# Chen-Suyi/PointRegGPT

Measured on AMD Instinct MI355X. Metric: generated point-cloud pairs/sec (node), 128x128 depth, 1000-step DDNM, higher is better.
Workload: dtype bf16; 1 GPU; configs[2]: full pipeline (SE(3) z-buffer reproject + MaskUnet + DDNM sampler + MaskUnet + f64 unproject); batch_per_gpu=64, image_size=128, transitions=1000, sampler=ancestral-ddnm, unet_dim=64, streams=2, parallelism=scene-sharded x1, no collectives, hipgraph=one captured transition (U-Net + update), replayed per step

## Files before the change

include/prg.h:

```cpp
#ifndef PRG_H
#define PRG_H

#include <stddef.h>
#include <stdint.h>

#ifdef __cplusplus
extern "C" {
#endif

#define PRG_ABI_VERSION 1

enum {
  PRG_OK = 0,
  PRG_E_INVALID = -1,
  PRG_E_HIP = -2,
  PRG_E_NOMEM = -3,
  PRG_E_STATE = -4
};

enum { PRG_F32 = 0, PRG_BF16 = 1, PRG_MXFP8 = 2, PRG_F16X3 = 3 };

int prg_abi_version(void);
const char* prg_last_error(void);
int prg_device_info(char* name, size_t name_len, int* compute_units);
// ... 17 lines not shown
                      int B, int H, int W, float depth_unit, float clip_lo, float clip_hi, void* stream);

int prg_depth_augment(const float* depth, float* out, int B, int H, int W, void* stream);

int prg_apply_mask(const float* prob, const float* depth, const uint8_t* hit, float thr, float* depth_out,
                   uint8_t* hit_out, float* img_cond, int B, int H, int W, void* stream);

int prg_occlusion_filter(const float* depth, const uint8_t* mask, float* out, int B, int H, int W, float threshold,
                         void* stream);

int prg_overlap_counts(const double* pts, const int64_t* offsets, int n_pairs, int64_t max_cloud, double radius,
                       int32_t* counts, void* stream);


typedef struct prg_unet prg_unet;

typedef struct prg_unet_config {
  int32_t dim;
  int32_t n_levels;
  int32_t dim_mults[8];
  int32_t in_channels;
  int32_t conditional;
  int32_t param_cond_dim;
  int32_t groups;
  int32_t sigmoid_out;
} prg_unet_config;

int64_t prg_unet_param_count(const prg_unet_config* cfg);

int prg_unet_create(const prg_unet_config* cfg, const float* weights, int64_t n_floats, int dtype,
                    prg_unet** out);
int prg_unet_destroy(prg_unet* h);
int prg_unet_set_time_freqs(prg_unet* h, const float* freqs, int n);
int prg_unet_reserve(prg_unet* h, int B, int S);

int prg_unet_forward(prg_unet* h, const float* x, const int64_t* time, const float* param_cond, float* out,
                     int B, int S, void* stream);
int prg_maskunet_forward(prg_unet* h, const float* depth, float* prob, int B, int S, void* stream);

int prg_unet_set_taps(prg_unet* h, int enable);
int prg_unet_get_tap(prg_unet* h, const char* name, float* out, int64_t out_capacity_floats, int* C, int* H,
                     int* W, void* stream);

int prg_debug_conv3x3(const float* x, const float* w, const float* bias, float* out, int B, int Cin, int Cout, int H, int W,
                      int dtype, void* stream);
int prg_debug_block_pair(const float* x, const float* w1, const float* b1, const float* gamma, const float* beta, const float* w2,
                         const float* b2, float* out, int B, int Cin, int C, int H, int W, int groups, int h16, void* stream);
int prg_debug_upsample_conv3x3(const float* x, const float* w, const float* bias, float* out, int B, int Cin, int Cout, int H,
                               int W, void* stream);
int prg_debug_conv4x4s2(const float* x, const float* w, const float* bias, float* out, int B, int Cin, int Cout, int H, int W,
                        void* stream);
int prg_debug_conv(const float* x, const float* w, const float* bias, float* out, int B, int Cin, int Cout, int H, int W,
                   int dtype, int K, int stride, void* stream);
int prg_debug_upsample_conv(const float* x, const float* w, const float* bias, float* out, int B, int Cin, int Cout, int H, int W,
                            int dtype, void* stream);


typedef struct prg_sampler prg_sampler;

typedef struct prg_step {
  int32_t t;
  int32_t clip_pred;
  float c_x0, c_x, c_eps, sigma;
  float sqrt_recip, sqrt_recipm1;
} prg_step;

int prg_sampler_create(prg_unet* unet, const prg_step* steps, int n_steps, int B, int S, prg_sampler** out);
int prg_sampler_destroy(prg_sampler* h);
int prg_sampler_set_graph(prg_sampler* h, int enable);

int prg_sampler_run(prg_sampler* h, const float* param_cond, const float* img_cond, const float* noise,
                    int64_t noise_slabs, const uint64_t* seeds, float* out, void* stream);

int prg_debug_sampler_step(float* x, const float* u, const float* img_cond, const uint64_t* seeds, const prg_step* step, int B,
                           int HW, int reps, float* avg_us, void* stream);

int prg_sampler_set_profile(prg_sampler* h, int enable);
int prg_sampler_get_profile(prg_sampler* h, double* conv_ms, int64_t* conv_launches, double* conv_flops,
                            double* total_ms);
int prg_sampler_get_profile_bytes(prg_sampler* h, double* conv_bytes);
int prg_sampler_get_profile_executed(prg_sampler* h, double* conv_flops_executed);
typedef struct prg_profile_shape {
  int32_t cin, cout, k, stride, ups, hout, wout;
  int32_t two_source, prologue;
  int32_t mx;
  int64_t launches;
  double ms, flops, flops_executed;
} prg_profile_shape;
int prg_sampler_get_profile_shapes(prg_sampler* h, prg_profile_shape* rows, int32_t max_rows, int32_t* n_rows);
int prg_sampler_get_profile_step(prg_sampler* h, double* step_ms, int64_t* step_launches);


int prg_host_crop_aabb(const double* pts, int64_t n, const double* lo, const double* hi, double* out, int64_t* n_out);
int prg_host_voxel_down_sample(const double* pts, int64_t n, double voxel, double* out, int64_t* n_out);
int prg_host_write_ply(const char* path, const double* pts, int64_t n);

typedef struct prg_pool prg_pool;
int prg_pool_create(int n_threads, prg_pool** out);
int prg_pool_destroy(prg_pool* p);
int prg_pool_wait(prg_pool* p, int64_t* jobs_done);
int prg_pool_submit_cloud(prg_pool* p, const char* path, const double* xyz, int64_t n, const uint8_t* valid,
                          const double* T_pre, int crop, const double* lo, const double* hi, double voxel,
                          const double* T_post);
int prg_pool_submit_image(prg_pool* p, const char* path, const float* img, int H, int W, int kind);
int prg_pool_submit_text(prg_pool* p, const char* path, const double* values, int rows, int cols);

// ... 5 lines not shown
```

pointreggpt_amd/_lib.py:

```python
from __future__ import annotations

import ctypes as C
import os
from pathlib import Path

_HERE = Path(__file__).resolve().parent
LIB_PATH = Path(os.environ.get("PRG_HIP_LIB", _HERE / "libprg_hip.so"))

PRG_F32, PRG_BF16, PRG_MXFP8, PRG_F16X3 = 0, 1, 2, 3


class PrgError(RuntimeError):
    pass


class UnetConfigC(C.Structure):
    _fields_ = [("dim", C.c_int32), ("n_levels", C.c_int32), ("dim_mults", C.c_int32 * 8),
                ("in_channels", C.c_int32), ("conditional", C.c_int32), ("param_cond_dim", C.c_int32),
                ("groups", C.c_int32), ("sigmoid_out", C.c_int32)]


class StepC(C.Structure):
    _fields_ = [("t", C.c_int32), ("clip_pred", C.c_int32), ("c_x0", C.c_float), ("c_x", C.c_float),
                ("c_eps", C.c_float), ("sigma", C.c_float), ("sqrt_recip", C.c_float),
                ("sqrt_recipm1", C.c_float)]


_P, _I, _F, _L = C.c_void_p, C.c_int, C.c_float, C.c_int64

PROTOTYPES = {
    "prg_abi_version": (C.c_int, []),
    "prg_last_error": (C.c_char_p, []),
    "prg_device_info": (C.c_int, [C.c_char_p, C.c_size_t, C.POINTER(C.c_int)]),
    "prg_depth2pc": (C.c_int, [_P, _P, _P, _P, _I, _I, _I, _F, _F, _F, _P]),
    "prg_pc2depth": (C.c_int, [_P, _P, _P, _P, _P, _I, _I, _I, _I, _P]),
    "prg_project_points_zbuffer": (C.c_int, [_P, _P, _P, _P, _P, _P, _I, _I, _I, _F, _P]),
    "prg_reproject_zbuffer": (C.c_int, [_P, _P, _P, _P, _P, _I, _I, _I, _F, _F, _F, _F, _P]),
    "prg_unproject_f64": (C.c_int, [_P, _P, _P, _P, _P, _I, _I, _I, _F, _F, _F, _P]),
    "prg_depth_augment": (C.c_int, [_P, _P, _I, _I, _I, _P]),
    "prg_apply_mask": (C.c_int, [_P, _P, _P, _F, _P, _P, _P, _I, _I, _I, _P]),
    "prg_occlusion_filter": (C.c_int, [_P, _P, _P, _I, _I, _I, _F, _P]),
    "prg_overlap_counts": (C.c_int, [_P, _P, _I, _L, C.c_double, _P, _P]),
    "prg_unet_param_count": (_L, [C.POINTER(UnetConfigC)]),
    "prg_unet_create": (C.c_int, [C.POINTER(UnetConfigC), _P, _L, _I, C.POINTER(_P)]),
    "prg_unet_destroy": (C.c_int, [_P]),
    "prg_unet_reserve": (C.c_int, [_P, _I, _I]),
    "prg_unet_set_time_freqs": (C.c_int, [_P, _P, _I]),
    "prg_unet_forward": (C.c_int, [_P, _P, _P, _P, _P, _I, _I, _P]),
    "prg_maskunet_forward": (C.c_int, [_P, _P, _P, _I, _I, _P]),
    "prg_debug_conv3x3": (C.c_int, [_P, _P, _P, _P, _I, _I, _I, _I, _I, _I, _P]),
    "prg_debug_block_pair": (C.c_int, [_P, _P, _P, _P, _P, _P, _P, _P, _I, _I, _I, _I, _I, _I, _I, _P]),
    "prg_debug_upsample_conv3x3": (C.c_int, [_P, _P, _P, _P, _I, _I, _I, _I, _I, _P]),
    "prg_debug_conv4x4s2": (C.c_int, [_P, _P, _P, _P, _I, _I, _I, _I, _I, _P]),
    "prg_debug_conv": (C.c_int, [_P, _P, _P, _P, _I, _I, _I, _I, _I, _I, _I, _I, _P]),
    "prg_debug_upsample_conv": (C.c_int, [_P, _P, _P, _P, _I, _I, _I, _I, _I, _I, _P]),
    "prg_unet_set_taps": (C.c_int, [_P, _I]),
    "prg_unet_get_tap": (C.c_int, [_P, C.c_char_p, _P, _L, C.POINTER(_I), C.POINTER(_I), C.POINTER(_I), _P]),
    "prg_sampler_create": (C.c_int, [_P, C.POINTER(StepC), _I, _I, _I, C.POINTER(_P)]),
    "prg_sampler_destroy": (C.c_int, [_P]),
    "prg_sampler_set_graph": (C.c_int, [_P, _I]),
    "prg_sampler_run": (C.c_int, [_P, _P, _P, _P, _L, _P, _P, _P]),
    "prg_sampler_set_profile": (C.c_int, [_P, _I]),
    "prg_sampler_get_profile": (C.c_int, [_P, C.POINTER(C.c_double), C.POINTER(_L), C.POINTER(C.c_double),
                                          C.POINTER(C.c_double)]),
    "prg_sampler_get_profile_bytes": (C.c_int, [_P, C.POINTER(C.c_double)]),
    "prg_sampler_get_profile_executed": (C.c_int, [_P, C.POINTER(C.c_double)]),
    "prg_sampler_get_profile_step": (C.c_int, [_P, C.POINTER(C.c_double), C.POINTER(_L)]),
    "prg_debug_sampler_step": (C.c_int, [_P, _P, _P, _P, _P, C.c_int, C.c_int, C.c_int, C.POINTER(C.c_float), _P]),
    "prg_sampler_get_profile_shapes": (C.c_int, [_P, _P, _I, C.POINTER(C.c_int32)]),
    "prg_host_crop_aabb": (C.c_int, [_P, _L, _P, _P, _P, C.POINTER(_L)]),
    "prg_host_voxel_down_sample": (C.c_int, [_P, _L, C.c_double, _P, C.POINTER(_L)]),
    "prg_host_write_ply": (C.c_int, [C.c_char_p, _P, _L]),
    "prg_pool_create": (C.c_int, [_I, C.POINTER(_P)]),
    "prg_pool_destroy": (C.c_int, [_P]),
    "prg_pool_wait": (C.c_int, [_P, C.POINTER(_L)]),
    "prg_pool_submit_cloud": (C.c_int, [_P, C.c_char_p, _P, _L, _P, _P, _I, _P, _P, C.c_double, _P]),
    "prg_pool_submit_image": (C.c_int, [_P, C.c_char_p, _P, _I, _I, _I]),
    "prg_pool_submit_text": (C.c_int, [_P, C.c_char_p, _P, _I, _I]),
}

_lib = None


def load():
    global _lib
    if _lib is not None:
        return _lib
    import torch
    if not LIB_PATH.exists():
        raise PrgError(f"{LIB_PATH} not found: build it with `python -c 'import __graft_entry__ as g; g.build()'` "
                       f"or `make -C pointreggpt_amd/csrc` (there is no CPU fallback)")
    try:
        lib = C.CDLL(str(LIB_PATH))
    except OSError as e:
        raise PrgError(f"cannot load {LIB_PATH}: {e}") from e
    lenient = os.environ.get("PRG_HIP_LIB_ALLOW_MISSING", "0") not in ("", "0") and bool(os.environ.get("PRG_HIP_LIB"))
    for name, (res, args) in PROTOTYPES.items():
        if lenient and not hasattr(lib, name):
            continue
        fn = getattr(lib, name)
        fn.restype = res
        fn.argtypes = args
    if lib.prg_abi_version() != 1:
        raise PrgError(f"ABI version mismatch: library {lib.prg_abi_version()}, binding 1")
    _lib = lib
    return lib
# ... 25 lines not shown
```

pointreggpt_amd/csrc/conv.h:

```cpp
#pragma once
#include <vector>

#include "common.h"

namespace prg {

template <typename T>
struct ConvTile {
  static constexpr int BK = 64 / (int)sizeof(T);
};

struct ConvDesc {
  int B, Hin, Win;
  int C0, C1;
  int ups;
  int KH, KW, stride, pad;
  int Hout, Wout;
  int Cout, CoutPad;
  int kchunks;
};

template <typename T>
void pack_conv_weight(const float* w_oihw, int Cout, int Cin, int KH, int KW, std::vector<T>& out, int* CoutPad,
                      int* kchunks);
// ... 44 lines not shown
}
typedef __attribute__((ext_vector_type(4))) unsigned int h16_u32x4;
#define PRG_H16_TRANS4(OP)                                                                                             \
  asm(OP "_e32 %0, %4\n\t" OP "_e32 %1, %5\n\t" OP "_e32 %2, %6\n\t" OP "_e32 %3, %7\n\t"                            \
      OP "_sdwa %0, %4 dst_sel:WORD_1 dst_unused:UNUSED_PRESERVE src0_sel:WORD_1\n\t"                                  \
      OP "_sdwa %1, %5 dst_sel:WORD_1 dst_unused:UNUSED_PRESERVE src0_sel:WORD_1\n\t"                                  \
      OP "_sdwa %2, %6 dst_sel:WORD_1 dst_unused:UNUSED_PRESERVE src0_sel:WORD_1\n\t"                                  \
      OP "_sdwa %3, %7 dst_sel:WORD_1 dst_unused:UNUSED_PRESERVE src0_sel:WORD_1\n\ts_nop 0"                           \
      : "=&v"(o0), "=&v"(o1), "=&v"(o2), "=&v"(o3)                                                                      \
      : "v"(i0), "v"(i1), "v"(i2), "v"(i3))
__device__ inline h16_u32x4 h16_silu8(h16_u32x4 x, const h16x2 (&a)[4], const h16x2 (&b)[4]) {
  const h16x2 nl2e = {(_Float16)-1.4426950408889634f, (_Float16)-1.4426950408889634f}, one = {(_Float16)1.0f, (_Float16)1.0f};
  h16x2 y[4];
  uint32_t i0, i1, i2, i3, o0, o1, o2, o3;
#pragma unroll
  for (int j = 0; j < 4; ++j) {
    const uint32_t w = x[j];
    y[j] = __builtin_elementwise_fma(__builtin_bit_cast(h16x2, w), a[j], b[j]);
  }
  i0 = __builtin_bit_cast(uint32_t, y[0] * nl2e); i1 = __builtin_bit_cast(uint32_t, y[1] * nl2e);
  i2 = __builtin_bit_cast(uint32_t, y[2] * nl2e); i3 = __builtin_bit_cast(uint32_t, y[3] * nl2e);
  PRG_H16_TRANS4("v_exp_f16");
  i0 = __builtin_bit_cast(uint32_t, __builtin_bit_cast(h16x2, o0) + one); i1 = __builtin_bit_cast(uint32_t, __builtin_bit_cast(h16x2, o1) + one);
  i2 = __builtin_bit_cast(uint32_t, __builtin_bit_cast(h16x2, o2) + one); i3 = __builtin_bit_cast(uint32_t, __builtin_bit_cast(h16x2, o3) + one);
  PRG_H16_TRANS4("v_rcp_f16");
  h16_u32x4 r;
  r[0] = __builtin_bit_cast(uint32_t, y[0] * __builtin_bit_cast(h16x2, o0));
  r[1] = __builtin_bit_cast(uint32_t, y[1] * __builtin_bit_cast(h16x2, o1));
  r[2] = __builtin_bit_cast(uint32_t, y[2] * __builtin_bit_cast(h16x2, o2));
  r[3] = __builtin_bit_cast(uint32_t, y[3] * __builtin_bit_cast(h16x2, o3));
  return r;
}
#undef PRG_H16_TRANS4
#endif

void pack_conv_weight_f16(const float* w_oihw, int Cout, int Cin, int KH, int KW, std::vector<uint16_t>& out);
bool conv_h16_pair_ok(const ConvLaunch<bf16_t>& L1, const ConvLaunch<bf16_t>& L2);

void pack_conv_weight_split(const float* w_oihw, int Cout, int Cin, int KH, int KW, std::vector<uint16_t>& out, int* CoutPad,
                            int* kchunks32, std::vector<float>* oscale = nullptr);
int try_launch_conv_split(const ConvLaunch<float>& L, hipStream_t s, int* gn_nsplit_out);

void s2d_equivalent_weights(const float* w_oihw, int Cout, int Cin, std::vector<float>& out);
void up_equivalent_weights(const float* w_oihw, int Cout, int Cin, std::vector<float>& out);

void pack_conv_weight_mxfp8(const float* w_oihw, int Cout, int Cin, int KH, int KW, std::vector<uint8_t>& data,
                            std::vector<uint8_t>& scales, int* CoutPad, int* chunks64);
uint8_t f32_to_e4m3(float v);
float e4m3_to_f32(uint8_t b);

template <typename T>
int launch_conv(const ConvLaunch<T>& L, hipStream_t s, int* gn_nsplit_out, int* acc_done = nullptr);

template <typename T>
bool conv_supports_prologue(const ConvDesc& d);

double conv_last_exec_scale();
int conv_last_was_mx();

inline double conv_flops(const ConvDesc& d) {
  return 2.0 * (double)d.B * d.Hout * d.Wout * d.Cout * (double)(d.C0 + d.C1) * d.KH * d.KW;
}

bool stem_conv_mfma_supported(int Cin, int Cout, int H, int W);
int launch_stem_conv_mfma(const float* x, const bf16_t* wf, const float* bias, bf16_t* out, int B, int Cin, int H, int W, hipStream_t s);
void pack_stem_mfma_weights(const float* w, int Cin, std::vector<bf16_t>& out);
int launch_stem_conv_mfma_split(const float* x, const uint16_t* wf, const float* bias, const float* wscale, float* out, int B, int Cin,
                                int H, int W, hipStream_t s);
void pack_stem_mfma_weights_split(const float* w, int Cin, std::vector<uint16_t>& out, std::vector<float>& scale);
template <typename T>
int launch_stem_conv(const float* x, const float* wk, const float* bias, T* out, int B, int Cin, int H, int W,
                     int Cout, hipStream_t s);

template <typename T>
int launch_head_conv(const T* x, const float* w, const float* bias, float* out, int64_t M, int C, int sigmoid,
                     hipStream_t s);

}
```

pointreggpt_amd/csrc/conv.hip:

```cpp
#include <cmath>
#include <cstdio>
#include <cstring>
#include <type_traits>

#include "blocks.h"
#include "conv.h"
#include "conv_epi.h"

namespace prg {

template <typename T>
struct Mma;

template <>
struct Mma<bf16_t> {
  static constexpr int UNITS_PER_CALL = 2;
  using Frag = bf16x8;
  __device__ static inline int unit_of(int call, int hi) { return call * 2 + hi; }
  __device__ static inline Frag load(const void* p) { return *reinterpret_cast<const Frag*>(p); }
  __device__ static inline void mma(const Frag& a, const Frag& b, f32x16& c, int ) {
    c = __builtin_amdgcn_mfma_f32_32x32x16_bf16(a, b, c, 0, 0, 0);
  }
};

// ... 725 lines not shown
  int rc;
  if ((rc = materialize_prologue(L, s))) return rc;
  if (hp.TH == 8 && hp.TW == 32 && hp.BN == 64) rc = launch_mx<8, 32, 64>(L, s, fuse, gn_nsplit_out);
  else if (hp.TH == 4 && hp.TW == 32 && hp.BN == 128) rc = launch_mx<4, 32, 128>(L, s, fuse, gn_nsplit_out);
  else if (hp.TH == 8 && hp.TW == 16 && hp.BN == 128) rc = launch_mx<8, 16, 128>(L, s, fuse, gn_nsplit_out);
  else if (hp.TH == 8 && hp.TW == 16 && hp.BN == 64) rc = launch_mx<8, 16, 64>(L, s, fuse, gn_nsplit_out);
  else return 0;
  if (rc == PRG_OK) g_last_mx = 1;
  return rc == PRG_OK ? 1 : rc;
}
static int try_mx(ConvLaunch<float>&, hipStream_t, int*, int*) { return 0; }

int try_launch_conv3x3_ws(const ConvLaunch<bf16_t>& L, hipStream_t s, int* gn_nsplit_out, int* acc_done);
int try_launch_conv3x3_c64(const ConvLaunch<bf16_t>& L, hipStream_t s, int* gn_nsplit_out, int* acc_done);
int try_launch_conv3x3_w256(const ConvLaunch<bf16_t>& L, hipStream_t s, int* gn_nsplit_out, int* acc_done);
int try_launch_conv4x4s2_w256(const ConvLaunch<bf16_t>& L, hipStream_t s);
int try_launch_conv3x3_up_w256(const ConvLaunch<bf16_t>& L, hipStream_t s);
static inline int try_down(const ConvLaunch<bf16_t>& L, hipStream_t s) { return try_launch_conv4x4s2_w256(L, s); }
static inline int try_down(const ConvLaunch<float>&, hipStream_t) { return 0; }
static inline int try_ws(ConvLaunch<bf16_t>& L, hipStream_t s, int* n, int* acc_done) {
  int r = try_launch_conv3x3_c64(L, s, n, acc_done);
  if (r == 0 && L.d.ups && !L.gn_partials) {
    r = try_launch_conv3x3_up_w256(L, s);
    if (r == 1) g_last_exec_scale = 4.0 / 9.0;
  }
  if (r == 0) r = try_launch_conv3x3_w256(L, s, n, acc_done);
  if (r != 0) return r;
  const ConvDesc& d = L.d;
  if (L.pro_fold.acc && d.KH == 3 && d.KW == 3 && d.stride == 1 && d.pad == 1 && d.C0 % 64 == 0 && d.C1 % 64 == 0 && d.Cout % 64 == 0)
    if (int rc = materialize_prologue(L, s)) return rc;
  return try_launch_conv3x3_ws(L, s, n, acc_done);
}
static inline int try_ws(ConvLaunch<float>&, hipStream_t, int*, int*) { return 0; }
static inline int try_split(const ConvLaunch<float>& L, hipStream_t s, int* n) { return try_launch_conv_split(L, s, n); }
static inline int try_split(const ConvLaunch<bf16_t>&, hipStream_t, int*) { return 0; }

bool conv_h16_pair_ok(const ConvLaunch<bf16_t>& L1in, const ConvLaunch<bf16_t>& L2in) {
  static const int on = env_int("PRG_H16", 1);
  if (!on) return false;
  ConvLaunch<bf16_t> L1 = L1in, L2 = L2in;
  auto mx_takes = [](const ConvLaunch<bf16_t>& L) { return L.w_mx && (L.d.Cout % 128 == 0 || mx_pure_env() || L.mx_pure); };
  if (mx_takes(L1) || mx_takes(L2) || !L2.w_f16 || !L1.gn_acc || !L2.pro_fold.acc) return false;
  L1.probe = L2.probe = 1;
  L1.out_f16 = 1;
  L2.in_f16 = 1;
  int ns = 0, ad = 0;
  int r1 = try_launch_conv3x3_c64(L1, nullptr, &ns, &ad);
  if (r1 == 0) r1 = try_launch_conv3x3_w256(L1, nullptr, &ns, &ad);
  if (r1 == 0) r1 = try_launch_conv3x3_ws(L1, nullptr, &ns, &ad);
  if (r1 != 1 || !ad) return false;
  int r2 = try_launch_conv3x3_c64(L2, nullptr, &ns, &ad);
  if (r2 == 0) r2 = try_launch_conv3x3_w256(L2, nullptr, &ns, &ad);
  return r2 == 1;
}

template <typename T>
int launch_conv(const ConvLaunch<T>& Lin, hipStream_t s, int* gn_nsplit_out, int* acc_done) {
  g_last_exec_scale = 1.0;
  g_last_mx = 0;
  if (acc_done) *acc_done = 0;
  ConvLaunch<T> L = Lin;
  const ConvDesc& d = L.d;
  constexpr int VEC = Elem<T>::kVec;
  PRG_CHECK(L.src0 && L.w && L.out, "conv: null pointer");
  PRG_CHECK(d.C0 % VEC == 0 && d.C1 % VEC == 0, "conv: channel counts must be multiples of the 16-byte vector");
  PRG_CHECK(d.C1 == 0 || L.src1, "conv: second source missing");
  PRG_CHECK(!L.res_a || (L.residual && L.res_b && d.KH == 1 && d.KW == 1 && d.Cout % 8 == 0),
            "conv: the activated residual is a 1x1 (implicit-GEMM, wide epilogue) feature");
  PRG_CHECK(!L.res_fold.acc || (L.residual && d.KH == 1 && d.KW == 1 && d.Cout % 8 == 0 && L.res_fold.cpg % 8 == 0 &&
                                L.res_fold.G * L.res_fold.cpg == d.Cout && L.res_fold.P && L.res_fold.Q),
            "conv: the folded activated residual needs a 1x1 conv whose 8-channel vectors lie inside one GroupNorm group");
  PRG_CHECK(d.CoutPad % 64 == 0 && d.CoutPad >= d.Cout, "conv: bad CoutPad");
  const int64_t M64 = (int64_t)d.B * d.Hout * d.Wout;
  PRG_CHECK(M64 > 0 && M64 < (int64_t)1 << 31, "conv: M out of range");
  const int M = (int)M64;
  const int want_stats = L.gn_partials != nullptr;
  if (gn_nsplit_out) *gn_nsplit_out = 0;
  {
    const int r = try_mx(L, s, gn_nsplit_out, acc_done);
    if (r < 0) return r;
    if (r == 1) return PRG_OK;
  }
  {
    int r = try_ws(L, s, gn_nsplit_out, acc_done);
    if (r == 0 && !L.gn_partials) r = try_down(L, s);
    if (r < 0) return r;
    if (r == 1) return PRG_OK;
  }
  PRG_CHECK(!L.out_f16 && !L.in_f16, "conv: an h16 launch reached a kernel without the f16 format (conv_h16_pair_ok disagrees with the dispatch)");
  if (int rc = materialize_prologue(L, s)) return rc;
  {
    const int r = try_split(L, s, gn_nsplit_out);
    if (r < 0) return r;
    if (r == 1) return PRG_OK;
  }
  HaloPick<T> hp;
  if (pick_halo<T>(d, &hp)) {
    const int cpg = L.gn_groups > 0 ? d.Cout / L.gn_groups : 0;
    const int tiles = (d.Wout / hp.TW) * (d.Hout / hp.TH);
    const int fuse = want_stats && cpg % 8 == 0 && cpg <= hp.BN && tiles <= kGnMaxSplit;
    if (hp.TH == 8 && hp.TW == 32 && hp.BN == 64) return launch_halo<T, 8, 32, 64>(L, s, fuse, gn_nsplit_out);
    if (hp.TH == 4 && hp.TW == 32 && hp.BN == 128) return launch_halo<T, 4, 32, 128>(L, s, fuse, gn_nsplit_out);
    if (hp.TH == 8 && hp.TW == 16 && hp.BN == 128) return launch_halo<T, 8, 16, 128>(L, s, fuse, gn_nsplit_out);
    if (hp.TH == 8 && hp.TW == 16 && hp.BN == 64) return launch_halo<T, 8, 16, 64>(L, s, fuse, gn_nsplit_out);
  }
  PRG_CHECK(!L.pro_a, "conv: fused prologue requested on a shape the halo kernel does not cover");
  if constexpr (std::is_same<T, bf16_t>::value) {
    if (d.CoutPad % 128 == 0 && M % 256 == 0 && (int64_t)(M / 256) * (d.CoutPad / 128) >= (int64_t)2 * 256)
      return launch_igemm<T, 256, 128>(L, M, s, want_stats, gn_nsplit_out);
  }
  if (d.CoutPad % 128 == 0) return launch_igemm<T, 128, 128>(L, M, s, want_stats, gn_nsplit_out);
  if (M >= 256 * 64) return launch_igemm<T, 256, 64>(L, M, s, want_stats, gn_nsplit_out);
  return launch_igemm<T, 128, 64>(L, M, s, want_stats, gn_nsplit_out);
}

void up_equivalent_weights(const float* w, int Cout, int Cin, std::vector<float>& out) {
  out.assign((size_t)4 * Cout * Cin * 4, 0.0f);
  auto slot = [](int dphase, int k) { const int r = dphase + k - 1; return (r >= 0 ? r / 2 : -1) - (dphase - 1); };
  for (int dy = 0; dy < 2; ++dy)
    for (int dx = 0; dx < 2; ++dx)
      for (int o = 0; o < Cout; ++o)
        for (int c = 0; c < Cin; ++c) {
          double acc[2][2] = {{0, 0}, {0, 0}};
          for (int ky = 0; ky < 3; ++ky)
            for (int kx = 0; kx < 3; ++kx) acc[slot(dy, ky)][slot(dx, kx)] += (double)w[(((size_t)o * Cin + c) * 3 + ky) * 3 + kx];
          float* dst = out.data() + ((((size_t)(2 * dy + dx) * Cout + o) * Cin + c) * 4);
          dst[0] = (float)acc[0][0]; dst[1] = (float)acc[0][1]; dst[2] = (float)acc[1][0]; dst[3] = (float)acc[1][1];
        }
}

void s2d_equivalent_weights(const float* w, int Cout, int Cin, std::vector<float>& out) {
  out.assign((size_t)Cout * 4 * Cin * 9, 0.0f);
  for (int o = 0; o < Cout; ++o)
    for (int c = 0; c < Cin; ++c)
      for (int ky = 0; ky < 4; ++ky)
        for (int kx = 0; kx < 4; ++kx) {
          const int by = ky >> 1, dy = ky & 1, bx = kx >> 1, dx = kx & 1;
          const int cv = (2 * dy + dx) * Cin + c;
          out[(((size_t)o * 4 * Cin + cv) * 3 + 1 + by) * 3 + 1 + bx] = w[(((size_t)o * Cin + c) * 4 + ky) * 4 + kx];
        }
}

template int launch_conv<float>(const ConvLaunch<float>&, hipStream_t, int*, int*);
template int launch_conv<bf16_t>(const ConvLaunch<bf16_t>&, hipStream_t, int*, int*);

template <typename T>
void pack_conv_weight(const float* w, int Cout, int Cin, int KH, int KW, std::vector<T>& out, int* CoutPad,
                      int* kchunks) {
  constexpr int BK = ConvTile<T>::BK;
  const int cp = (Cout + 63) / 64 * 64;
  const int kcn = (Cin + BK - 1) / BK;
  out.assign((size_t)KH * KW * kcn * cp * BK, Elem<T>::store(0.0f));
  for (int kh = 0; kh < KH; ++kh)
    for (int kw = 0; kw < KW; ++kw)
      for (int kc = 0; kc < kcn; ++kc)
        for (int n = 0; n < Cout; ++n)
          for (int k = 0; k < BK; ++k) {
            int c = kc * BK + k;
            if (c >= Cin) break;
            float v = w[(((size_t)n * Cin + c) * KH + kh) * KW + kw];
            out[((((size_t)(kh * KW + kw)) * kcn + kc) * cp + n) * BK + k] = Elem<T>::store(v);
          }
  *CoutPad = cp;
  *kchunks = kcn;
}
template void pack_conv_weight<float>(const float*, int, int, int, int, std::vector<float>&, int*, int*);
// ... 362 lines not shown
```

pointreggpt_amd/csrc/unet.hip:

```cpp
#include <algorithm>
#include <cmath>
#include <cstdlib>
#include <cstring>
#include <map>
#include <memory>
#include <string>
#include <type_traits>
#include <vector>

#include "blocks.h"
#include "conv.h"
#include "sampler.h"

namespace prg {

static thread_local std::string g_err;
void set_error(const std::string& m) { g_err = m; }
int device_cu_count() {
  static std::atomic<int> cus[64];
  int dev = 0;
  if (hipGetDevice(&dev) != hipSuccess) return 0;
  std::atomic<int>& c = cus[dev & 63];
  int n = c.load(std::memory_order_acquire);
  if (n <= 0) {
// ... 1551 lines not shown
  L1.src0 = reinterpret_cast<const bf16_t*>(d_x); L1.w = reinterpret_cast<const bf16_t*>(d_w1); L1.bias = reinterpret_cast<const float*>(d_b1);
  L1.out = reinterpret_cast<bf16_t*>(d_h);
  L1.gn_partials = reinterpret_cast<float*>(d_part); L1.gn_acc = reinterpret_cast<long long*>(d_acc);
  desc(L2, C, cp2, kc2);
  L2.src0 = reinterpret_cast<const bf16_t*>(d_h); L2.w = reinterpret_cast<const bf16_t*>(d_w2); L2.w_f16 = reinterpret_cast<const uint16_t*>(d_w2h);
  L2.bias = reinterpret_cast<const float*>(d_b2); L2.out = reinterpret_cast<bf16_t*>(d_y);
  GnFold f{};
  f.acc = reinterpret_cast<const long long*>(d_acc); f.P = reinterpret_cast<const float*>(d_pq); f.Q = f.P + C; f.pq_stride = 0;
  f.G = groups; f.cpg = C / groups; f.inv_n = 1.0f / ((float)(H * W) * (float)f.cpg);
  L2.pro_fold = f;
  L2.pro_a = reinterpret_cast<const float*>(d_coef); L2.pro_b = L2.pro_a + (size_t)B * C;
  if (rc == PRG_OK && h16) {
    if (!conv_h16_pair_ok(L1, L2)) rc = fail(PRG_E_INVALID, "prg_debug_block_pair: the kernels this shape dispatches to do not implement the f16 format");
    L1.out_f16 = 1;
    L2.in_f16 = 1;
  }
  int ns = 0, ad = 0;
  if (rc == PRG_OK) rc = launch_conv<bf16_t>(L1, s, &ns, &ad);
  if (rc == PRG_OK && !ad) rc = fail(PRG_E_INVALID, "prg_debug_block_pair: conv1's kernel does not accumulate fixed-point statistics for this shape");
  if (rc == PRG_OK) rc = launch_conv<bf16_t>(L2, s, nullptr);
  if (rc == PRG_OK) rc = launch_nhwc_to_nchw_f32<bf16_t>(reinterpret_cast<const bf16_t*>(d_y), out, B, H * W, C, s);
  if (hipStreamSynchronize(s) != hipSuccess && rc == PRG_OK) rc = fail(PRG_E_HIP, "prg_debug_block_pair: stream synchronise failed");
  cleanup();
  return rc;
}

int prg_debug_conv3x3(const float* x, const float* w, const float* bias, float* out, int B, int Cin, int Cout, int H, int W,
                      int dtype, void* stream) {
  return debug_conv(x, w, bias, out, B, Cin, Cout, H, W, dtype, 3, 1, stream);
}

int prg_debug_conv(const float* x, const float* w, const float* bias, float* out, int B, int Cin, int Cout, int H, int W,
                   int dtype, int K, int stride, void* stream) {
  PRG_CHECK((K == 1 || K == 3 || K == 4) && (stride == 1 || stride == 2), "prg_debug_conv: K must be 1, 3 or 4, stride 1 or 2");
  PRG_CHECK(dtype == PRG_F32 || dtype == PRG_F16X3 || K != 1, "prg_debug_conv: 1x1 convs only in the float32-storage modes");
  PRG_CHECK(stride == 1 || (H % 2 == 0 && W % 2 == 0), "prg_debug_conv: odd image size");
  return debug_conv(x, w, bias, out, B, Cin, Cout, H, W, dtype, K, stride, stream);
}

int prg_debug_upsample_conv3x3(const float* x, const float* w, const float* bias, float* out, int B, int Cin, int Cout, int H, int W,
                               void* stream) {
  return debug_conv(x, w, bias, out, B, Cin, Cout, H, W, PRG_BF16, 3, 1, stream, 1);
}

int prg_debug_upsample_conv(const float* x, const float* w, const float* bias, float* out, int B, int Cin, int Cout, int H, int W,
                            int dtype, void* stream) {
  return debug_conv(x, w, bias, out, B, Cin, Cout, H, W, dtype, 3, 1, stream, 1);
}

int prg_debug_conv4x4s2(const float* x, const float* w, const float* bias, float* out, int B, int Cin, int Cout, int H, int W,
                        void* stream) {
  PRG_CHECK(H % 2 == 0 && W % 2 == 0, "prg_debug_conv4x4s2: odd image size");
  return debug_conv(x, w, bias, out, B, Cin, Cout, H, W, PRG_BF16, 4, 2, stream);
}

int prg_sampler_create(prg_unet* unet, const prg_step* steps, int n_steps, int B, int S, prg_sampler** out) {
  PRG_CHECK(unet && steps && out, "prg_sampler_create: null pointer");
  PRG_CHECK(unet->lay.cfg.conditional && unet->lay.cfg.in_channels == 1, "prg_sampler_create: needs the conditional U-Net");
  PRG_CHECK(n_steps > 0 && B > 0 && S > 0, "prg_sampler_create: bad sizes");
  int rc = reserve(unet, B, S);
  if (rc) return rc;
  std::unique_ptr<prg_sampler> h(new prg_sampler());
  h->unet = unet; h->B = B; h->S = S; h->n_steps = n_steps;
  h->steps.assign(steps, steps + n_steps);
  const Layout& L = unet->lay;
  const int e = L.emb, d0 = L.cfg.dim, W = L.ss_total;
  const size_t HW = (size_t)S * S;
  const int R = n_steps > B ? n_steps : B;
  if (hipMalloc(&h->d_steps, sizeof(prg_step) * n_steps) != hipSuccess ||
      hipMalloc(&h->d_tpart, sizeof(float) * (size_t)n_steps * W) != hipSuccess ||
      hipMalloc(&h->d_ppart, sizeof(float) * (size_t)B * W) != hipSuccess ||
      hipMalloc(&h->d_scratch, sizeof(float) * (size_t)R * (d0 + 2 * e) + sizeof(int32_t) * n_steps) != hipSuccess ||
      hipMalloc(&h->d_x, sizeof(float) * B * HW) != hipSuccess || hipMalloc(&h->d_u, sizeof(float) * B * HW) != hipSuccess ||
      hipMalloc(&h->d_step, 2 * sizeof(int)) != hipSuccess || hipMalloc(&h->d_seeds, sizeof(uint64_t) * B) != hipSuccess)
    return fail(PRG_E_NOMEM, "prg_sampler_create: hipMalloc failed");
  PRG_HIP(hipMemcpy(h->d_steps, steps, sizeof(prg_step) * n_steps, hipMemcpyHostToDevice));
  PRG_HIP(hipStreamCreateWithFlags(&h->own_stream, hipStreamDefault));
  {
    hipStream_t s = h->own_stream;
    float* sinu = h->d_scratch;
    float* h1 = sinu + (size_t)R * d0;
    float* temb = h1 + (size_t)R * e;
    int32_t* tdev = reinterpret_cast<int32_t*>(temb + (size_t)R * e);
    std::vector<int32_t> tt(n_steps);
    for (int k = 0; k < n_steps; ++k) tt[k] = steps[k].t;
    PRG_HIP(hipMemcpyAsync(tdev, tt.data(), sizeof(int32_t) * n_steps, hipMemcpyHostToDevice, s));
    const float* F = unet->d_flat;
    if ((rc = launch_sinusoidal_i32(tdev, unet->d_freqs, sinu, n_steps, d0, s))) return rc;
    if ((rc = launch_linear(sinu, d0, 0, F + L.tm1_w, d0, 0, F + L.tm1_b, h1, e, n_steps, d0, e, ACT_NONE, ACT_GELU, s))) return rc;
    if ((rc = launch_linear(h1, e, 0, F + L.tm3_w, e, 0, F + L.tm3_b, temb, e, n_steps, e, e, ACT_NONE, ACT_NONE, s))) return rc;
    auto one = [&](const ResP& r) -> int {
      return launch_linear(temb, e, 0, F + r.mlp_w, 2 * e, 0, F + r.mlp_b, h->d_tpart + r.ss_off, W, n_steps, e,
                           2 * r.cout, ACT_SILU, ACT_NONE, s);
    };
    for (auto& lv : L.downs) { if ((rc = one(lv.r0))) return rc; if ((rc = one(lv.r1))) return rc; }
    for (auto& lv : L.ups) { if ((rc = one(lv.r0))) return rc; if ((rc = one(lv.r1))) return rc; }
    if ((rc = one(L.mid1))) return rc;
    if ((rc = one(L.mid2))) return rc;
    if ((rc = one(L.fin))) return rc;
    PRG_HIP(hipStreamSynchronize(s));
  }
  *out = h.release();
  return PRG_OK;
}

int prg_sampler_destroy(prg_sampler* h) {
// ... 161 lines not shown
```

Measured before the change: 14.49 pairs/s.

## Add dedicated async-LDS MFMA GEMM kernel for 1x1 convolutions

Adds a specialised bf16 GEMM kernel for 1x1 stride-1 convolutions, including two-source concatenated inputs. It uses global_load_lds double buffering into swizzled LDS, 32x32x16 MFMA tiles, and a fused bias/residual/GN-SiLU epilogue. The conv dispatcher tries it before the generic implicit-GEMM path when enough tiles exist and no stats or prologue are needed, aiming to cut the im2col-style overhead of the generic kernel on 1x1 shapes. A debug entry point is added to compare both paths. The risk is lower occupancy from 64KB of LDS, and coverage is limited to shapes whose channel counts are multiples of 64 and 128.

```diff
diff --git a/include/prg.h b/include/prg.h
--- a/include/prg.h
+++ b/include/prg.h
@@ -93,6 +93,8 @@
                         void* stream);
 int prg_debug_conv(const float* x, const float* w, const float* bias, float* out, int B, int Cin, int Cout, int H, int W,
                    int dtype, int K, int stride, void* stream);
+int prg_debug_conv1x1(const float* x0, const float* x1, const float* w, const float* bias, const float* residual, const float* res_ab,
+                      float* out, int B, int C0, int C1, int Cout, int H, int W, int path, void* stream);
 int prg_debug_upsample_conv(const float* x, const float* w, const float* bias, float* out, int B, int Cin, int Cout, int H, int W,
                             int dtype, void* stream);
 
diff --git a/pointreggpt_amd/_lib.py b/pointreggpt_amd/_lib.py
--- a/pointreggpt_amd/_lib.py
+++ b/pointreggpt_amd/_lib.py
@@ -52,6 +52,7 @@
     "prg_debug_block_pair": (C.c_int, [_P, _P, _P, _P, _P, _P, _P, _P, _I, _I, _I, _I, _I, _I, _I, _P]),
     "prg_debug_upsample_conv3x3": (C.c_int, [_P, _P, _P, _P, _I, _I, _I, _I, _I, _P]),
     "prg_debug_conv4x4s2": (C.c_int, [_P, _P, _P, _P, _I, _I, _I, _I, _I, _P]),
+    "prg_debug_conv1x1": (C.c_int, [_P, _P, _P, _P, _P, _P, _P, _I, _I, _I, _I, _I, _I, _I, _P]),
     "prg_debug_conv": (C.c_int, [_P, _P, _P, _P, _I, _I, _I, _I, _I, _I, _I, _I, _P]),
     "prg_debug_upsample_conv": (C.c_int, [_P, _P, _P, _P, _I, _I, _I, _I, _I, _I, _P]),
     "prg_unet_set_taps": (C.c_int, [_P, _I]),
diff --git a/pointreggpt_amd/csrc/conv.h b/pointreggpt_amd/csrc/conv.h
--- a/pointreggpt_amd/csrc/conv.h
+++ b/pointreggpt_amd/csrc/conv.h
@@ -120,6 +120,8 @@
 template <typename T>
 int launch_conv(const ConvLaunch<T>& L, hipStream_t s, int* gn_nsplit_out, int* acc_done = nullptr);
 
+int launch_conv1x1_path(const ConvLaunch<bf16_t>& L, hipStream_t s, int path);
+
 template <typename T>
 bool conv_supports_prologue(const ConvDesc& d);
 
diff --git a/pointreggpt_amd/csrc/conv.hip b/pointreggpt_amd/csrc/conv.hip
--- a/pointreggpt_amd/csrc/conv.hip
+++ b/pointreggpt_amd/csrc/conv.hip
@@ -801,6 +801,20 @@
   int r2 = try_launch_conv3x3_c64(L2, nullptr, &ns, &ad);
   if (r2 == 0) r2 = try_launch_conv3x3_w256(L2, nullptr, &ns, &ad);
   return r2 == 1;
+}
+
+int try_launch_conv_gemm(const ConvLaunch<bf16_t>& L, hipStream_t s, int force);
+
+template <typename T>
+static int launch_generic_igemm(const ConvLaunch<T>& L, int M, hipStream_t s, int want_stats, int* gn_nsplit_out) {
+  const ConvDesc& d = L.d;
+  if constexpr (std::is_same<T, bf16_t>::value) {
+    if (d.CoutPad % 128 == 0 && M % 256 == 0 && (int64_t)(M / 256) * (d.CoutPad / 128) >= (int64_t)2 * 256)
+      return launch_igemm<T, 256, 128>(L, M, s, want_stats, gn_nsplit_out);
+  }
+  if (d.CoutPad % 128 == 0) return launch_igemm<T, 128, 128>(L, M, s, want_stats, gn_nsplit_out);
+  if (M >= 256 * 64) return launch_igemm<T, 256, 64>(L, M, s, want_stats, gn_nsplit_out);
+  return launch_igemm<T, 128, 64>(L, M, s, want_stats, gn_nsplit_out);
 }
 
 template <typename T>
@@ -855,12 +869,28 @@
   }
   PRG_CHECK(!L.pro_a, "conv: fused prologue requested on a shape the halo kernel does not cover");
   if constexpr (std::is_same<T, bf16_t>::value) {
-    if (d.CoutPad % 128 == 0 && M % 256 == 0 && (int64_t)(M / 256) * (d.CoutPad / 128) >= (int64_t)2 * 256)
-      return launch_igemm<T, 256, 128>(L, M, s, want_stats, gn_nsplit_out);
-  }
-  if (d.CoutPad % 128 == 0) return launch_igemm<T, 128, 128>(L, M, s, want_stats, gn_nsplit_out);
-  if (M >= 256 * 64) return launch_igemm<T, 256, 64>(L, M, s, want_stats, gn_nsplit_out);
-  return launch_igemm<T, 128, 64>(L, M, s, want_stats, gn_nsplit_out);
+    const int r = want_stats ? 0 : try_launch_conv_gemm(L, s, 0);
+    if (r < 0) return r;
+    if (r == 1) return PRG_OK;
+  }
+  return launch_generic_igemm<T>(L, M, s, want_stats, gn_nsplit_out);
+}
+
+int launch_conv1x1_path(const ConvLaunch<bf16_t>& L, hipStream_t s, int path) {
+  const ConvDesc& d = L.d;
+  PRG_CHECK(L.src0 && L.w && L.out && (d.C1 == 0 || L.src1), "conv1x1: null pointer");
+  PRG_CHECK(d.KH == 1 && d.KW == 1 && d.stride == 1 && d.pad == 0 && !d.ups && d.C0 % 8 == 0 && d.C1 % 8 == 0 && d.Cout % 8 == 0,
+            "conv1x1: not a 1x1 / stride 1 convolution of 8-channel multiples");
+  PRG_CHECK(path == 0 || path == 1, "conv1x1: path must be 0 (conv_igemm_kernel) or 1 (conv_gemm_kernel)");
+  const int64_t M64 = (int64_t)d.B * d.Hout * d.Wout;
+  PRG_CHECK(M64 > 0 && M64 < (int64_t)1 << 31, "conv1x1: M out of range");
+  g_last_exec_scale = 1.0;
+  g_last_mx = 0;
+  if (path == 0) return launch_generic_igemm<bf16_t>(L, (int)M64, s, 0, nullptr);
+  const int r = try_launch_conv_gemm(L, s, 1);
+  if (r < 0) return r;
+  PRG_CHECK(r == 1, "conv1x1: shape not covered by conv_gemm_kernel");
+  return PRG_OK;
 }
 
 void up_equivalent_weights(const float* w, int Cout, int Cin, std::vector<float>& out) {
diff --git a/pointreggpt_amd/csrc/conv_gemm.hip b/pointreggpt_amd/csrc/conv_gemm.hip
--- /dev/null
+++ b/pointreggpt_amd/csrc/conv_gemm.hip
@@ -0,0 +1,198 @@
+#include <atomic>
+
+#include "conv_epi.h"
+
+namespace prg {
+
+__global__ __launch_bounds__(256, 2) void conv_gemm_kernel(const ConvLaunch<bf16_t> L, const int tiles_m, const int tiles_n) {
+  constexpr int NW = 4;
+  constexpr int BM = 128, BN = 128, ROWB = 128;
+  constexpr int TM = 2;
+  constexpr int APW = BM / 8 / NW, BPW = BN / 8 / NW;
+  constexpr int TILEB = (BM + BN) * ROWB;
+
+  extern __shared__ __attribute__((aligned(16))) char smem[];
+  float* const stage = reinterpret_cast<float*>(smem);
+
+  const ConvDesc& d = L.d;
+  const int lin = xcd_remap(blockIdx.x, tiles_m * tiles_n);
+  const int tn = lin % tiles_n, tm = lin / tiles_n;
+  const int tid = threadIdx.x, wave = tid >> 6, lane = tid & 63;
+  const int l31 = lane & 31, hi = lane >> 5;
+  const int wm = wave >> 1, wn = wave & 1;
+
+  const char* asrc0[APW];
+  const char* asrc1[APW];
+  int bsrc[BPW];
+#pragma unroll
+  for (int r = 0; r < APW; ++r) {
+    const int row = (wave * APW + r) * 8 + (lane >> 3);
+    const int u = (lane & 7) ^ ((row >> 1) & 7);
+    const int64_t m = (int64_t)tm * BM + row;
+    asrc0[r] = reinterpret_cast<const char*>(L.src0 + m * d.C0 + u * 8);
+    asrc1[r] = d.C1 ? reinterpret_cast<const char*>(L.src1 + m * d.C1 + u * 8) : asrc0[r];
+  }
+#pragma unroll
+  for (int r = 0; r < BPW; ++r) {
+    const int n = (wave * BPW + r) * 8 + (lane >> 3);
+    const int u = (lane & 7) ^ ((n >> 1) & 7);
+    bsrc[r] = (((u >> 2) * d.CoutPad + tn * BN + n) * 32 + (u & 3) * 8) * 2;
+  }
+  const char* const wbase = reinterpret_cast<const char*>(L.w);
+  const size_t wstep = (size_t)d.CoutPad * 128;
+  const int t0 = d.C0 >> 6;
+  const int nt = (d.C0 + d.C1) >> 6;
+
+  auto stage_tile = [&](int t, int buf) {
+    const bool first = t < t0;
+    const int aoff = (first ? t : t - t0) * 128;
+    char* const Ab = smem + buf * TILEB + wave * (APW * 8 * ROWB);
+    char* const Bb = smem + buf * TILEB + BM * ROWB + wave * (BPW * 8 * ROWB);
+    const char* const wt = wbase + (size_t)t * wstep;
+#pragma unroll
+    for (int r = 0; r < APW; ++r)
+      __builtin_amdgcn_global_load_lds((const __attribute__((address_space(1))) void*)((first ? asrc0[r] : asrc1[r]) + aoff),
+                                       (__attribute__((address_space(3))) void*)(Ab + r * 8 * ROWB), 16, 0, 0);
+#pragma unroll
+    for (int r = 0; r < BPW; ++r)
+      __builtin_amdgcn_global_load_lds((const __attribute__((address_space(1))) void*)(wt + bsrc[r]),
+                                       (__attribute__((address_space(3))) void*)(Bb + r * 8 * ROWB), 16, 0, 0);
+  };
+
+  f32x16 acc[TM][2];
+#pragma unroll
+  for (int i = 0; i < TM; ++i)
+#pragma unroll
+    for (int j = 0; j < 2; ++j)
+#pragma unroll
+      for (int e = 0; e < 16; ++e) acc[i][j][e] = 0.0f;
+
+  const int key = (l31 >> 1) & 7;
+  const int aoffs = (wm * 64 + l31) * ROWB, boffs = BM * ROWB + (wn * 64 + l31) * ROWB;
+
+  stage_tile(0, 0);
+  typedef __attribute__((ext_vector_type(4))) unsigned int u32x4;
+  const int cc = lane & 7, rr = lane >> 3;
+  const int col = tn * BN + wn * 64 + cc * 8;
+  const int64_t mrow0 = (int64_t)tm * BM + wm * 64 + rr;
+  float bias[8];
+#pragma unroll
+  for (int u = 0; u < 8; ++u) bias[u] = (L.bias ? L.bias : reinterpret_cast<const float*>(L.w))[col + u];
+  if (!L.bias)
+#pragma unroll
+    for (int u = 0; u < 8; ++u) bias[u] = 0.0f;
+  const bool has_res = L.residual != nullptr;
+  const bool act = L.res_a != nullptr || L.res_fold.acc != nullptr;
+  u32x4 rv[TM * 4];
+#pragma unroll
+  for (int k = 0; k < TM * 4; ++k)
+    rv[k] = *reinterpret_cast<const u32x4*>(has_res ? L.residual + (mrow0 + k * 8) * d.Cout + col : L.out);
+  float fa[8], fb[8];
+  if (has_res && act) {
+    const int img = (int)mrow0 / (d.Hout * d.Wout);
+    if (L.res_fold.acc) {
+      const GnFold& f = L.res_fold;
+      float mean, rstd;
+      gn_fold_stats(f, img, col / f.cpg, mean, rstd);
+      const float* pp = f.P + (size_t)img * f.pq_stride + col;
+      const float* pq = f.Q + (size_t)img * f.pq_stride + col;
+#pragma unroll
+      for (int u = 0; u < 8; ++u) {
+        fa[u] = rstd * pp[u];
+        fb[u] = fmaf(-mean, fa[u], pq[u]);
+      }
+    } else {
+      const size_t cb = (size_t)img * d.Cout + col;
+      const float4 a0 = *reinterpret_cast<const float4*>(L.res_a + cb), a1 = *reinterpret_cast<const float4*>(L.res_a + cb + 4);
+      const float4 b0 = *reinterpret_cast<const float4*>(L.res_b + cb), b1 = *reinterpret_cast<const float4*>(L.res_b + cb + 4);
+      fa[0] = a0.x; fa[1] = a0.y; fa[2] = a0.z; fa[3] = a0.w; fa[4] = a1.x; fa[5] = a1.y; fa[6] = a1.z; fa[7] = a1.w;
+      fb[0] = b0.x; fb[1] = b0.y; fb[2] = b0.z; fb[3] = b0.w; fb[4] = b1.x; fb[5] = b1.y; fb[6] = b1.z; fb[7] = b1.w;
+    }
+  }
+
+  for (int t = 0; t < nt; ++t) {
+    asm volatile("s_waitcnt vmcnt(0) lgkmcnt(0)\n\ts_barrier" ::: "memory");
+    if (t + 1 < nt) stage_tile(t + 1, (t + 1) & 1);
+    const char* const Ab = smem + (t & 1) * TILEB + aoffs;
+    const char* const Bb = smem + (t & 1) * TILEB + boffs;
+#pragma unroll
+    for (int g = 0; g < 4; ++g) {
+      const int uo = ((2 * g + hi) ^ key) << 4;
+      bf16x8 fa[TM], fb[2];
+#pragma unroll
+      for (int i = 0; i < TM; ++i) fa[i] = *reinterpret_cast<const bf16x8*>(Ab + i * 32 * ROWB + uo);
+#pragma unroll
+      for (int j = 0; j < 2; ++j) fb[j] = *reinterpret_cast<const bf16x8*>(Bb + j * 32 * ROWB + uo);
+#pragma unroll
+      for (int i = 0; i < TM; ++i)
+#pragma unroll
+        for (int j = 0; j < 2; ++j) acc[i][j] = __builtin_amdgcn_mfma_f32_32x32x16_bf16(fa[i], fb[j], acc[i][j], 0, 0, 0);
+    }
+  }
+
+  constexpr int P = 68;
+  float* const st = stage + wave * 32 * P;
+  asm volatile("s_waitcnt lgkmcnt(0)\n\ts_barrier" ::: "memory");
+#pragma unroll
+  for (int i = 0; i < TM; ++i) {
+#pragma unroll
+    for (int j = 0; j < 2; ++j)
+#pragma unroll
+      for (int e = 0; e < 16; ++e) st[((e & 3) + 8 * (e >> 2) + 4 * hi) * P + j * 32 + l31] = acc[i][j][e];
+    asm volatile("s_waitcnt lgkmcnt(0)" ::: "memory");
+#pragma unroll
+    for (int pass = 0; pass < 4; ++pass) {
+      const int r = pass * 8 + rr;
+      const int64_t m = mrow0 + i * 32 + pass * 8;
+      const float4 v0 = *reinterpret_cast<const float4*>(st + r * P + cc * 8);
+      const float4 v1 = *reinterpret_cast<const float4*>(st + r * P + cc * 8 + 4);
+      float v[8] = {v0.x, v0.y, v0.z, v0.w, v1.x, v1.y, v1.z, v1.w};
+#pragma unroll
+      for (int u = 0; u < 8; ++u) v[u] += bias[u];
+      if (has_res) {
+        const u32x4 w = rv[i * 4 + pass];
+        float rres[8];
+#pragma unroll
+        for (int u = 0; u < 8; ++u) rres[u] = __uint_as_float((u & 1) ? (w[u >> 1] & 0xffff0000u) : (w[u >> 1] << 16));
+        if (act) {
+#pragma unroll
+          for (int u = 0; u < 8; ++u) v[u] += Elem<bf16_t>::silu(fmaf(rres[u], fa[u], fb[u]));
+        } else {
+#pragma unroll
+          for (int u = 0; u < 8; ++u) v[u] += rres[u];
+        }
+      }
+      Vec16<bf16_t> o;
+#pragma unroll
+      for (int u = 0; u < 8; ++u) o.e[u] = Elem<bf16_t>::store(v[u]);
+      vec_store(L.out + m * d.Cout + col, o);
+    }
+    asm volatile("s_waitcnt lgkmcnt(0)" ::: "memory");
+  }
+}
+
+int try_launch_conv_gemm(const ConvLaunch<bf16_t>& L, hipStream_t s, int force) {
+  constexpr int BM = 128, BN = 128;
+  const ConvDesc& d = L.d;
+  if (!(d.KH == 1 && d.KW == 1 && d.stride == 1 && d.pad == 0 && !d.ups)) return 0;
+  if (d.C0 <= 0 || d.C0 % 64 || d.C1 % 64 || d.Cout % BN || d.CoutPad != d.Cout || d.kchunks * 32 != d.C0 + d.C1) return 0;
+  if (L.pro_a || L.pro_fold.acc || L.in_f16 || L.out_f16 || L.gn_partials || L.probe) return 0;
+  const int64_t M = (int64_t)d.B * d.Hout * d.Wout;
+  if (M <= 0 || M % BM || d.Hin != d.Hout || d.Win != d.Wout || (d.Hout * d.Wout) % 64) return 0;
+  const int64_t tiles = M / BM * (d.Cout / BN);
+  if (tiles >= (int64_t)1 << 31) return 0;
+  if (!force && tiles < 256) return 0;
+  constexpr size_t kLds = (size_t)2 * (BM + BN) * 128;
+  static_assert(kLds >= (size_t)4 * 32 * 68 * sizeof(float), "the epilogue's scratch lives in the operand buffers");
+  static DeviceOnce attr_done;
+  if (!attr_done.done()) {
+    PRG_HIP(hipFuncSetAttribute(reinterpret_cast<const void*>(&conv_gemm_kernel), hipFuncAttributeMaxDynamicSharedMemorySize, (int)kLds));
+    attr_done.mark();
+  }
+  const int tiles_m = (int)(M / BM), tiles_n = d.Cout / BN;
+  conv_gemm_kernel<<<dim3((unsigned)tiles), 256, kLds, s>>>(L, tiles_m, tiles_n);
+  PRG_LAUNCH_CHECK();
+  return 1;
+}
+
+}
diff --git a/pointreggpt_amd/csrc/unet.hip b/pointreggpt_amd/csrc/unet.hip
--- a/pointreggpt_amd/csrc/unet.hip
+++ b/pointreggpt_amd/csrc/unet.hip
@@ -1627,6 +1627,52 @@
                         void* stream) {
   PRG_CHECK(H % 2 == 0 && W % 2 == 0, "prg_debug_conv4x4s2: odd image size");
   return debug_conv(x, w, bias, out, B, Cin, Cout, H, W, PRG_BF16, 4, 2, stream);
+}
+
+int prg_debug_conv1x1(const float* x0, const float* x1, const float* w, const float* bias, const float* residual, const float* res_ab,
+                      float* out, int B, int C0, int C1, int Cout, int H, int W, int path, void* stream) {
+  PRG_CHECK(x0 && w && out && (C1 == 0 || x1), "prg_debug_conv1x1: null pointer");
+  PRG_CHECK(B > 0 && H > 0 && W > 0 && C0 > 0 && C1 >= 0 && C0 % 8 == 0 && C1 % 8 == 0 && Cout > 0 && Cout % 8 == 0, "prg_debug_conv1x1: bad shape");
+  PRG_CHECK(path == 0 || path == 1, "prg_debug_conv1x1: path must be 0 or 1");
+  PRG_CHECK(!res_ab || residual, "prg_debug_conv1x1: res_ab needs a residual");
+  hipStream_t s = (hipStream_t)stream;
+  const size_t M = (size_t)B * H * W;
+  std::vector<bf16_t> packed;
+  int cp = 0, kc = 0;
+  pack_conv_weight<bf16_t>(w, Cout, C0 + C1, 1, 1, packed, &cp, &kc);
+  std::vector<float> zb(Cout, 0.0f);
+  void *d_x0 = nullptr, *d_x1 = nullptr, *d_out = nullptr, *d_w = nullptr, *d_b = nullptr, *d_ab = nullptr;
+  auto cleanup = [&]() { for (void* p : {d_x0, d_x1, d_out, d_w, d_b, d_ab}) if (p) (void)hipFree(p); };
+  if (hipMalloc(&d_x0, M * C0 * 2) != hipSuccess || (C1 && hipMalloc(&d_x1, M * C1 * 2) != hipSuccess) ||
+      hipMalloc(&d_out, M * Cout * 2) != hipSuccess || hipMalloc(&d_w, packed.size() * 2) != hipSuccess || hipMalloc(&d_b, Cout * 4) != hipSuccess ||
+      (res_ab && hipMalloc(&d_ab, (size_t)2 * B * Cout * 4) != hipSuccess)) {
+    cleanup();
+    return fail(PRG_E_NOMEM, "prg_debug_conv1x1: hipMalloc failed");
+  }
+  if (hipMemcpy(d_w, packed.data(), packed.size() * 2, hipMemcpyHostToDevice) != hipSuccess ||
+      hipMemcpy(d_b, bias ? bias : zb.data(), Cout * 4, hipMemcpyHostToDevice) != hipSuccess ||
+      (res_ab && hipMemcpy(d_ab, res_ab, (size_t)2 * B * Cout * 4, hipMemcpyHostToDevice) != hipSuccess)) {
+    cleanup();
+    return fail(PRG_E_HIP, "prg_debug_conv1x1: hipMemcpy failed");
+  }
+  int rc = launch_nchw_f32_to_nhwc<bf16_t>(x0, reinterpret_cast<bf16_t*>(d_x0), B, H * W, C0, s);
+  if (rc == PRG_OK && C1) rc = launch_nchw_f32_to_nhwc<bf16_t>(x1, reinterpret_cast<bf16_t*>(d_x1), B, H * W, C1, s);
+  if (rc == PRG_OK && residual) rc = launch_nchw_f32_to_nhwc<bf16_t>(residual, reinterpret_cast<bf16_t*>(d_out), B, H * W, Cout, s);
+  if (rc == PRG_OK) {
+    ConvLaunch<bf16_t> L{};
+    L.d.B = B; L.d.Hin = H; L.d.Win = W; L.d.C0 = C0; L.d.C1 = C1; L.d.ups = 0; L.d.KH = 1; L.d.KW = 1; L.d.stride = 1; L.d.pad = 0;
+    L.d.Hout = H; L.d.Wout = W; L.d.Cout = Cout; L.d.CoutPad = cp; L.d.kchunks = kc;
+    L.src0 = reinterpret_cast<const bf16_t*>(d_x0); L.src1 = reinterpret_cast<const bf16_t*>(d_x1);
+    L.w = reinterpret_cast<const bf16_t*>(d_w); L.bias = reinterpret_cast<const float*>(d_b); L.out = reinterpret_cast<bf16_t*>(d_out);
+    L.gn_groups = 8;
+    if (residual) L.residual = L.out;
+    if (res_ab) { L.res_a = reinterpret_cast<const float*>(d_ab); L.res_b = L.res_a + (size_t)B * Cout; }
+    rc = launch_conv1x1_path(L, s, path);
+  }
+  if (rc == PRG_OK) rc = launch_nhwc_to_nchw_f32<bf16_t>(reinterpret_cast<const bf16_t*>(d_out), out, B, H * W, Cout, s);
+  if (hipStreamSynchronize(s) != hipSuccess && rc == PRG_OK) rc = fail(PRG_E_HIP, "prg_debug_conv1x1: stream synchronise failed");
+  cleanup();
+  return rc;
 }
 
 int prg_sampler_create(prg_unet* unet, const prg_step* steps, int n_steps, int B, int S, prg_sampler** out) {
```

After: 14.48 pairs/s. No clear change (-0.1%).
